# OpenGene/gencore

Measured on AMD Instinct MI355X. Metric: consensus read-pairs/sec (whole node) + clustering HBM GB/s vs roofline, higher is better.
Workload: dtype u8

## Files before the change

### gencore_amd/csrc/engine.hip

```cpp
#include <hip/hip_runtime.h>
#include <hip/hip_ext.h>
#include <cstdio>
#include <cstdlib>
#include <algorithm>
#include <cstring>
#include <ctime>
#include <string>
#include <vector>

#include "gce_kernels.hpp"
#include "gce_pair2.hpp"
#include "gce_vote.hpp"
#include "gce_deep.hpp"
#include "gce_output.hpp"
#include "gce_depth.hpp"
#include "gce_inflate.hpp"
#include "gce_deflate.hpp"

namespace {

static thread_local double t_alloc_s = 0.0; static thread_local long t_alloc_n = 0; static thread_local size_t t_alloc_bytes = 0;
static inline double mono_s() { struct timespec ts; clock_gettime(CLOCK_MONOTONIC, &ts); return (double)ts.tv_sec + 1e-9 * (double)ts.tv_nsec; }
long long g_dev_live = 0, g_dev_peak = 0;
static int64_t g_pass_idx_ctr[4] = {0, 0, 0, 0};
// ... 680 lines not shown
    }
    p.n_ref = nref; p.ref_data = e->d_ref_ptr.as<const uint8_t *>(); p.ref_len = e->d_ref_len.as<int64_t>(); p.ref_win = win.empty() ? nullptr : e->d_ref_win.as<int64_t>();

    Work w{};
    const int64_t n_sblk = (N + SB_READS - 1) / SB_READS;
    w.n_sblk = n_sblk;
    const int64_t max_events = e->have_tick ? (int64_t)e->h_ev_tid.size() + 2 : (p.tick_offset % p.period + N) / p.period + 2;
    w.max_events = (int)max_events;
    uint64_t T = ((uint64_t)n1 + (uint64_t)n1 / 4 + 2 * SCAN_TILE - 1) / SCAN_TILE * SCAN_TILE;
    w.tsize = T; w.tinv = 1.0 / (double)T;
    {
        uint64_t genome = 0; for (uint32_t v : e->target_len) genome += v;
        const uint64_t qmax = (genome * TAB_WAYS + TAB_WAYS) / T + 1;
        int cb = 1; while (cb < 33 && (1ull << cb) <= (uint64_t)N + 1024) cb++;
        int qb = 1; while (qb < 52 && (1ull << qb) <= qmax) qb++;
        p.nw_cb = cb; p.nw_bd = 62 - cb - qb; p.nw_ok = !e->target_len.empty() && p.nw_bd >= 1;
        if (p.nw_bd > 40) p.nw_bd = 40;
    }
    const size_t qual_bytes = hb.qual_bytes ? hb.qual_bytes : 1;
    const size_t nsb1 = (size_t)(n_sblk > 0 ? n_sblk : 1);
#define ENS(buf, bytes) HIPCHK(e->buf.ensure(bytes))
    ENS(uinfo, n1 * 8); ENS(rdesc, n1 * sizeof(ReadDescP)); ENS(spatch, n1 * 4); ENS(slot, n1 * 4 + 16); ENS(score, qual_bytes + 64);
    ENS(out_flag, n1 + 144);        ENS(nmx, n1 * 4); ENS(orec, n1 * sizeof(OutRec)); ENS(out_index, n1 * 4);
    ENS(lrec, nsb1 * SB_READS * sizeof(LeadRec)); ENS(lout, nsb1 * SB_READS * sizeof(LeadOut));
    ENS(bhdr, nsb1 * sizeof(BlkHdr)); ENS(blk_base, nsb1 * 4);
    ENS(ev_tid, (size_t)max_events * 4); ENS(ev_pos, (size_t)max_events * 4); ENS(ev_read, (size_t)max_events * 4);
    ENS(table, T * sizeof(TabEntry)); ENS(toff, T * 4);
    ENS(k64, n1 * 24); ENS(members, n1 * 4); ENS(sorted, n1 * 4); ENS(pl, n1 * 4); ENS(pr, n1 * 4); ENS(pu, n1 * 4); ENS(pg, n1 * 4); ENS(gpl, n1 * 4); ENS(gpr, n1 * 4);
    ENS(grp_begin, n1 * 4); ENS(grp_n, n1 * 4); ENS(slow_list, n1 * 4 + 64);
    w.slow_list = e->slow_list.as<uint32_t>();
    ENS(deep_list, (n1 / 64 + 64) * 16); w.deep_list = e->deep_list.p;
    const unsigned nblk_N = cdiv(n1, SCAN_TILE);
    ENS(scan_part, std::max<size_t>(2 * nsb1, (size_t)2 * nblk_N) * 8 + 16);     ENS(si, sizeof(StreamInfo));
    w.uinfo = e->uinfo.as<uint64_t>(); w.rdesc = e->rdesc.as<ReadDescP>(); w.spatch = e->spatch.as<uint32_t>();
    w.slot = e->slot.as<uint32_t>(); w.score = e->score.as<int8_t>();
    w.out_flag = e->out_flag.as<uint8_t>(); w.nmx = e->nmx.as<uint32_t>(); w.orec = e->orec.as<OutRec>(); w.out_index = e->out_index.as<uint32_t>();
    w.lrec = e->lrec.as<LeadRec>(); w.lout = e->lout.as<LeadOut>(); w.bhdr = e->bhdr.as<BlkHdr>(); w.blk_base = e->blk_base.as<uint32_t>();
    w.ev_tid = e->ev_tid.as<int32_t>(); w.ev_pos = e->ev_pos.as<int32_t>(); w.ev_read = e->ev_read.as<uint32_t>();
    w.tab = e->table.as<TabEntry>(); w.toff = e->toff.as<uint32_t>();
    w.k64 = e->k64.as<uint64_t>(); w.members = e->members.as<uint32_t>(); w.sorted = e->sorted.as<uint32_t>(); w.pl = e->pl.as<uint32_t>(); w.pr = e->pr.as<uint32_t>();
    w.pu = e->pu.as<uint32_t>(); w.pg = e->pg.as<uint32_t>(); w.gpl = e->gpl.as<uint32_t>(); w.gpr = e->gpr.as<uint32_t>();
    w.grp_begin = e->grp_begin.as<uint32_t>(); w.grp_n = e->grp_n.as<uint32_t>();
    w.scan_part = e->scan_part.as<uint64_t>(); w.si = e->si.as<StreamInfo>();
    ENS(cl_ikey, n1 * 4); ENS(cl_start, n1 * 4); ENS(cl_n, n1 * 4);
    w.cl_ikey = e->cl_ikey.as<uint32_t>(); w.cl_start = e->cl_start.as<uint32_t>(); w.cl_n = e->cl_n.as<uint32_t>();

    StreamInfo init{}; init.first_unmapped = NONE32; init.err_key = ~0ull; init.lq_min = 0x7FFFFFFF; init.lq_max = -1;
    if (e->have_tick) { init.n_events = init.n_events_a = (int)e->h_ev_tid.size(); }
    HIPCHK(hipMemcpyAsync(e->si.p, &init, sizeof init, hipMemcpyHostToDevice, e->stream));
    if (e->have_tick && !e->h_ev_tid.empty()) {
        HIPCHK(hipMemcpyAsync(e->ev_tid.p, e->h_ev_tid.data(), e->h_ev_tid.size() * 4, hipMemcpyHostToDevice, e->stream));
        HIPCHK(hipMemcpyAsync(e->ev_pos.p, e->h_ev_pos.data(), e->h_ev_pos.size() * 4, hipMemcpyHostToDevice, e->stream));
    }
    hipStream_t s = e->stream;
    if (!e->tab_clean || e->tab_clean_ptr != e->table.p || e->tab_clean_cap != e->table.cap) {
        HIPCHK(hipMemsetAsync(e->table.p, 0, e->table.cap, s));
        e->tab_clean_ptr = e->table.p; e->tab_clean_cap = e->table.cap;
    }
    e->tab_clean = false;
    HIPCHK(hipEventRecord(e->ev[EV_START], s));
    HIPCHK(hipMemsetAsync(e->out_flag.p, 0, n1, s));
    if (N > 0) LAUNCH_EV(k_cluster, dim3((unsigned)n_sblk), dim3(SB_T), s, e->ev[EV_CLUSTER], b, p, w);
#ifdef CL_PROF
    if (N > 0) {
        StreamInfo hs; (void)hipStreamSynchronize(s); (void)hipMemcpy(&hs, e->si.p, sizeof hs, hipMemcpyDeviceToHost);
        static const char *nm[3] = {"key records + keys", "LDS leaders", "stores"};
        const double blocks = (double)hs.prof[15];
        fprintf(stderr, "k_cluster phases, mean per block (us), %.0f blocks:", blocks);
        for (int k = 0; k < 3; k++) fprintf(stderr, " %s %.2f;", nm[k], blocks ? hs.prof[k] / blocks / 100.0 : 0.0);
        fprintf(stderr, "\n");
    }
#endif
    if (N <= 0) HIPCHK(hipEventRecord(e->ev[EV_CLUSTER], s));
    CANARY("EV_CLUSTER");
    if (N > 0) {
        if (!e->have_tick) {
            hipLaunchKernelGGL(k_blk_scan, dim3(1), dim3(1024), 0, s, w, p);
            hipLaunchKernelGGL(k_events, dim3(cdiv(max_events, EV_T / 64)), dim3(EV_T), 0, s, b, p, w);
        }
        const unsigned nb4 = cdiv(n_sblk, 4);
        hipLaunchKernelGGL(k_leaders, dim3(nb4), dim3(256), 0, s, b, p, w);
        hipLaunchKernelGGL(k_num_reduce, dim3(nb4), dim3(256), 0, s, w, p.nw_cb);
        hipLaunchKernelGGL(k_scan_partials, dim3(1), dim3(1024), 0, s, w.scan_part, (uint64_t)nb4, &w.si->n_clusters, (unsigned long long *)nullptr);
        hipLaunchKernelGGL(k_num_apply, dim3(nb4), dim3(256), 0, s, w);
        LAUNCH_EV(k_scatter, dim3((unsigned)n_sblk), dim3(SB_T), s, e->ev[EV_CSR], N, w);
    } else HIPCHK(hipEventRecord(e->ev[EV_CSR], s));
    CANARY("EV_CSR");
    unsigned long long si_seq1 = 0;
    if ((rc = read_si_begin(e, &si_seq1)) != GCE_OK) return rc;
    if (N > 0) {
#ifndef GCE_DESCRIBE_BLOCKS
#define GCE_DESCRIBE_BLOCKS 32768
#endif
        const int64_t n_tiles = (N + 255) / 256;
        int tpb = (int)((n_tiles + GCE_DESCRIBE_BLOCKS - 1) / GCE_DESCRIBE_BLOCKS); if (tpb < 1) tpb = 1;
        LAUNCH_EV(k_describe, dim3(cdiv(n_tiles, tpb)), dim3(256), s, e->ev[EV_DESCRIBE], b, p, w, tpb);
    } else HIPCHK(hipEventRecord(e->ev[EV_DESCRIBE], s));
    CANARY("EV_DESCRIBE");
    if ((rc = read_si_end(e, si_seq1)) != GCE_OK) return rc;
    HIPCHK(hipGetLastError());
    e->tab_clean = true;
    const uint32_t C = (uint32_t)e->h_si.n_clusters;
    const size_t c1 = C ? C : 1;
    ENS(cl_npairs, c1 * 4); ENS(cl_ngroups, c1 * 4); ENS(cl_gbase, c1 * 4); ENS(cl_nresult, c1 * 4); ENS(cl_hasumi, c1); ENS(cl_tier, c1);
    w.cl_npairs = e->cl_npairs.as<uint32_t>(); w.cl_ngroups = e->cl_ngroups.as<uint32_t>(); w.cl_gbase = e->cl_gbase.as<uint32_t>();
    w.cl_nresult = e->cl_nresult.as<uint32_t>(); w.cl_hasumi = e->cl_hasumi.as<uint8_t>(); w.cl_tier = e->cl_tier.as<uint8_t>();
    uint32_t NG = 0;
    bool si_behind_describe = false;
    if (C > 0 && e->dev_error == 0) {
        ENS(left_list, c1 * 4 + 64); w.left_list = e->left_list.as<uint32_t>();
        ENS(pf_flag, c1 + 64); ENS(pf_list, c1 * 4); ENS(pq_flag, c1 + 64); ENS(pq_list, c1 * 4); ENS(p16_flag, c1 + 64); ENS(p16_list, c1 * 4);
        w.pf_flag = e->pf_flag.as<uint8_t>(); w.pf_list = e->pf_list.as<uint32_t>(); w.pq_flag = e->pq_flag.as<uint8_t>(); w.pq_list = e->pq_list.as<uint32_t>(); w.p16_flag = e->p16_flag.as<uint8_t>(); w.p16_list = e->p16_list.as<uint32_t>();
        const bool pair_classes = (double)N > 10.0 * (double)C;
        if (!pair_classes) fill_many(s, {FillSeg{e->pf_flag.p, c1, 0u, 0u}, FillSeg{e->pq_flag.p, c1, 0u, 0u}});
        const unsigned nbc = cdiv(C, SCAN_TILE);
        auto compact = [&](uint8_t *flag, uint32_t *list, unsigned long long *count) {
            hipLaunchKernelGGL(k_flag_reduce, dim3(nbc), dim3(256), 0, s, (const uint8_t *)flag, (uint64_t)C, w.scan_part);
            hipLaunchKernelGGL(k_scan_partials, dim3(1), dim3(1024), 0, s, w.scan_part, (uint64_t)nbc, count, (unsigned long long *)nullptr);
            hipLaunchKernelGGL(k_flag_apply, dim3(nbc), dim3(256), 0, s, (const uint8_t *)flag, (uint64_t)C, (const uint64_t *)w.scan_part, list);
        };
#ifdef PS_STOP
        {
            hipEvent_t a_, b_, c_; (void)hipEventCreate(&a_); (void)hipEventCreate(&b_); (void)hipEventCreate(&c_);
            (void)hipEventRecord(a_, s);
            hipLaunchKernelGGL(k_pairing_sub<16>, dim3(cdiv(C, 4 * WAVES_PER_BLOCK)), dim3(256), 0, s, b, p, w, C, (const uint32_t *)nullptr, (const unsigned long long *)nullptr, w.pq_flag, 0);
            (void)hipEventRecord(b_, s);
            hipLaunchKernelGGL(k_pairing_sub<32>, dim3(cdiv(C, 2 * WAVES_PER_BLOCK)), dim3(256), 0, s, b, p, w, C, (const uint32_t *)nullptr, (const unsigned long long *)nullptr, w.pf_flag, 0);
            (void)hipEventRecord(c_, s); (void)hipEventSynchronize(c_);
            float m1 = 0, m2 = 0; (void)hipEventElapsedTime(&m1, a_, b_); (void)hipEventElapsedTime(&m2, b_, c_);
            fprintf(stderr, "k_pairing_sub up to tick %d: <16> %.3f ms, <32> over ALL clusters %.3f ms\n", PS_STOP, m1, m2);
            return fail(e, GCE_ERR_INVALID, "experiment build");
        }
#endif
        ENS(pd_slab, PD_BIG_BLOCKS * PD_SLAB);
        if (pair_classes) {
            hipLaunchKernelGGL(k_pair_class_reduce, dim3(nbc), dim3(256), 0, s, (const uint32_t *)w.cl_n, C, w.scan_part);
            hipLaunchKernelGGL(k_scan_partials, dim3(1), dim3(1024), 0, s, w.scan_part, (uint64_t)nbc, &w.si->n_p16_items, &w.si->n_pq_items);
            hipLaunchKernelGGL(k_pair_class_apply, dim3(nbc), dim3(256), 0, s, (const uint32_t *)w.cl_n, C, (const uint64_t *)w.scan_part, w.p16_list, w.pq_list, w.pf_list, w.si);
            static const bool tiers_aux = getenv("GCE_NO_AUX_STREAM") == nullptr;
            hipStream_t s2 = s;
            if (tiers_aux) {
                if ((rc = aux_ready(e)) != GCE_OK) return rc;
                s2 = e->aux_stream;
                HIPCHK(hipEventRecord(e->aux_ev[0], s));
                HIPCHK(hipStreamWaitEvent(s2, e->aux_ev[0], 0));
            }
            hipLaunchKernelGGL(k_pairing_fast, dim3(2048), dim3(256), 0, s2, b, p, w, C, (const uint32_t *)w.pf_list);
            hipLaunchKernelGGL(k_pairing_deep<false>, dim3(256), dim3(PD_T), 0, s2, b, p, w, (uint8_t *)nullptr);
            if (tiers_aux) HIPCHK(hipEventRecord(e->aux_ev[1], s2));
            hipLaunchKernelGGL(k_pairing_sub<16>, dim3(cdiv(C, 4 * WAVES_PER_BLOCK)), dim3(256), 0, s, b, p, w, C, (const uint32_t *)w.p16_list, (const unsigned long long *)&w.si->n_p16_items, w.pq_flag, 1);
            hipLaunchKernelGGL(k_pairing_sub<32>, dim3(cdiv(C, 2 * WAVES_PER_BLOCK)), dim3(256), 0, s, b, p, w, C, (const uint32_t *)w.pq_list, (const unsigned long long *)&w.si->n_pq_items, w.pf_flag, 1);
            if (tiers_aux) HIPCHK(hipStreamWaitEvent(s, e->aux_ev[1], 0));
        } else {
            hipLaunchKernelGGL(k_pairing_sub<16>, dim3(cdiv(C, 4 * WAVES_PER_BLOCK)), dim3(256), 0, s, b, p, w, C, (const uint32_t *)nullptr, (const unsigned long long *)nullptr, w.pq_flag, 0);
            compact(w.pq_flag, w.pq_list, &w.si->n_pq_items);
            hipLaunchKernelGGL(k_pairing_sub<32>, dim3(cdiv(C, 2 * WAVES_PER_BLOCK)), dim3(256), 0, s, b, p, w, C, (const uint32_t *)w.pq_list, (const unsigned long long *)&w.si->n_pq_items, w.pf_flag, 0);
            compact(w.pf_flag, w.pf_list, &w.si->n_pf_items);
            hipLaunchKernelGGL(k_pairing_fast, dim3(2048), dim3(256), 0, s, b, p, w, C, (const uint32_t *)w.pf_list);
            hipLaunchKernelGGL(k_pairing_deep<false>, dim3(256), dim3(PD_T), 0, s, b, p, w, (uint8_t *)nullptr);
        }
        hipLaunchKernelGGL(k_pairing_deep<true>, dim3(PD_BIG_BLOCKS), dim3(PD_T), 0, s, b, p, w, e->pd_slab.as<uint8_t>());
        hipLaunchKernelGGL(k_pairing_slow<0>, dim3(1024), dim3(256), 0, s, b, p, w);
        hipLaunchKernelGGL(k_pairing_slow<1>, dim3(1024, 16), dim3(256), 0, s, b, p, w);
        hipLaunchKernelGGL(k_pairing_slow<2>, dim3(1024), dim3(256), 0, s, b, p, w);
        const unsigned nblk_C = cdiv(C, SCAN_TILE);
        hipLaunchKernelGGL(k_scan_reduce, dim3(nblk_C), dim3(256), 0, s, (const uint32_t *)w.cl_ngroups, (uint64_t)C, w.scan_part);
        hipLaunchKernelGGL(k_scan_partials, dim3(1), dim3(1024), 0, s, w.scan_part, (uint64_t)nblk_C, &w.si->n_pairs , &w.si->n_groups);
        hipLaunchKernelGGL(k_u32_apply, dim3(nblk_C), dim3(256), 0, s, (const uint32_t *)w.cl_ngroups, w.cl_gbase, (uint64_t)C, (const uint64_t *)w.scan_part);
        ENS(gl_cluster, n1 * 4); ENS(g_begin, n1 * 4); ENS(g_np, n1 * 4); ENS(gw, n1 * 8); ENS(g_wbase, n1 * 4);
        const size_t vb_cap = ((VB_MINW + 3) * n1) / VB_W + 8;
        ENS(vb_start, vb_cap * 4);
        w.gl_cluster = e->gl_cluster.as<uint32_t>(); w.g_begin = e->g_begin.as<uint32_t>(); w.g_np = e->g_np.as<uint32_t>();
        w.gw = e->gw.as<uint64_t>(); w.g_wbase = e->g_wbase.as<uint32_t>(); w.vb_start = e->vb_start.as<uint32_t>();
        HIPCHK(hipMemsetAsync(e->vb_start.p, 0xFF, vb_cap * 4, s));
        hipLaunchKernelGGL(k_group_fill, dim3(cdiv(C, 256)), dim3(256), 0, s, w, C, p.skip_low_complexity_thr, (uint32_t)VB_W, (uint32_t)VB_MINW);
        hipLaunchKernelGGL(k_u64_reduce, dim3(nblk_N), dim3(256), 0, s, (const uint64_t *)w.gw, (const unsigned long long *)&w.si->n_groups, w.scan_part);
        hipLaunchKernelGGL(k_u64_partials, dim3(1), dim3(1024), 0, s, w.scan_part, (const unsigned long long *)&w.si->n_groups, &w.si->vote_weight);
        LAUNCH_EV(k_vote_batches, dim3(nblk_N), dim3(256), s, e->ev[EV_PAIRING], w, (const unsigned long long *)&w.si->n_groups, (const uint64_t *)w.scan_part);
        CANARY("EV_PAIRING");
        if ((rc = read_si(e)) != GCE_OK) return rc;
// ... 350 lines not shown
```

### gencore_amd/csrc/gce_cluster.hpp

```cpp
#pragma once

#ifndef SB_T
#define SB_T 512
#endif
#ifndef SB_U
#define SB_U 2
#endif
#define SB_READS (SB_T * SB_U)
#define SB_LDS_SLOTS (2 * SB_READS)
#define SB_OFF_BITS (SB_READS == 1024 ? 10 : 9)
static_assert(SB_READS == 512 || SB_READS == 1024, "LeadRec.info packs a place and a count of SB_READS");

struct __attribute__((aligned(16))) LeadRec { unsigned long long kw; uint32_t info, runlen; };
static_assert(sizeof(LeadRec) == 16, "LeadRec must stay 16 bytes");
#define LI_ODD (1u << 22)
struct __attribute__((aligned(8))) BlkHdr { uint32_t n_lead, n_clu; };
struct __attribute__((aligned(8))) LeadOut { uint32_t h, rb; };
#define LO_OWNER 0x80000000u

__device__ __forceinline__ uint32_t d_thr_mode(uint32_t ikey, const StreamInfo *si, const DevParams &p) {
    uint32_t inst = ikey & 0x7FFFFFFFu, seg_b = ikey >> 31;
    if (!seg_b) {
        if ((int)(inst + 1) <= si->n_events_a) return THR_PROPER;
        if (si->first_unmapped != NONE32) return THR_UNPROPER;
        return p.trailing_flush ? THR_PROPER : THR_UNPROPER;
    }
    return ((int)(inst + 1) <= si->n_events) ? THR_PROPER : THR_NEVER;
}

struct __attribute__((aligned(16))) TabEntry { unsigned long long key; unsigned long long ic; };
static_assert(sizeof(TabEntry) == 16, "TabEntry must stay 16 bytes");
#define TAB_OCC (1ull << 63)
#define TAB_EXO (1ull << 62)

#define TAB_WAYS 8
__device__ __forceinline__ uint64_t d_tab_index(const ClusterKey &k, uint32_t ikey, const DevParams &p) {
    uint64_t g = (k.tid >= 0 && k.tid < p.n_targets && p.target_cum) ? p.target_cum[k.tid] : (uint64_t)(uint32_t)k.tid * 0x9E3779B97F4A7C15ull;
    uint64_t m = ((uint64_t)k.right * 0x165667B19E3779F9ull) ^ ((uint64_t)ikey * 0xD6E8FEB86659FD93ull);
    m ^= m >> 29;
    return (((g + (uint64_t)(uint32_t)k.left) & 0x0000FFFFFFFFFFFFull) * TAB_WAYS) | (m & (TAB_WAYS - 1));
}
__device__ __forceinline__ unsigned long long d_pack_key(const ClusterKey &k, const DevParams &p) {
    const long long delta1 = k.right - (long long)k.left + 1;
    const int bd = 62 - p.key_bt - p.key_bl;
    if (k.tid >= 0 && ((uint64_t)(uint32_t)k.tid >> p.key_bt) == 0 && k.left >= 0 && ((uint64_t)(uint32_t)k.left >> p.key_bl) == 0 &&
        delta1 >= 0 && bd > 0 && ((uint64_t)delta1 >> bd) == 0)
        return TAB_OCC | (uint64_t)(uint32_t)k.tid | ((uint64_t)(uint32_t)k.left << p.key_bt) | ((uint64_t)delta1 << (p.key_bt + p.key_bl));
    return 0ull;
}
__device__ __forceinline__ ClusterKey d_unpack_key(unsigned long long kw, const DevParams &p) {
    ClusterKey k;
    k.tid = (int32_t)(kw & ((1ull << p.key_bt) - 1ull));
    k.left = (int32_t)((kw >> p.key_bt) & ((1ull << p.key_bl) - 1ull));
    const long long delta1 = (long long)((kw & ~(TAB_OCC | TAB_EXO)) >> (p.key_bt + p.key_bl));
    k.right = (long long)k.left + delta1 - 1;
    return k;
}
__device__ __forceinline__ unsigned long long d_exotic_key(uint32_t ikey, uint32_t read) {
    return TAB_OCC | TAB_EXO | ((uint64_t)((ikey & 0x1FFFFFFFu) | ((ikey >> 31) << 29)) << 32) | read;
}

#ifdef CL_PROF
#define CL_TICK(k) do { if (threadIdx.x == 0 && (blockIdx.x & 31) == 0) { const unsigned long long now_ = wall_clock64(); atomicAdd(&w.si->prof[k], now_ - t_prev_); t_prev_ = now_; } } while (0)
#else
#define CL_TICK(k) do { } while (0)
#endif
__global__ __launch_bounds__(SB_T, 2048 / SB_T) void k_cluster(DevBatch b, DevParams p, Work w) {
    __shared__ uint32_t s_slot[SB_LDS_SLOTS];
    __shared__ unsigned long long s_kw[SB_READS];
    __shared__ uint32_t s_cnt[SB_READS];
    __shared__ uint16_t s_num[SB_READS];
    __shared__ uint32_t s_wcnt[SB_U][SB_T / 64];
    __shared__ uint32_t s_nlead;
    __shared__ uint32_t s_unm[SB_T / 64];
    const int lane = lane_id(), wv = threadIdx.x >> 6;
#ifdef CL_PROF
    unsigned long long t_prev_ = wall_clock64();
    if (threadIdx.x == 0 && (blockIdx.x & 31) == 0) atomicAdd(&w.si->prof[15], 1ull);
#endif
    int64_t idx[SB_U]; gce_core k[SB_U]; int2 pv[SB_U];
#pragma unroll
    for (int u = 0; u < SB_U; u++) {
        idx[u] = ((int64_t)blockIdx.x * SB_U + u) * SB_T + threadIdx.x;
        union { gce_core c; uint4 q[2]; } t;
        t.q[0] = make_uint4(0, 0, 0, 0); t.q[1] = t.q[0];
        pv[u] = make_int2(-1, -1);
        if (idx[u] < b.n) {
            const uint4 *src = reinterpret_cast<const uint4 *>(b.core + idx[u]); t.q[0] = src[0]; t.q[1] = src[1];
            if (idx[u] > 0) pv[u] = *reinterpret_cast<const int2 *>(b.core + idx[u] - 1);
        }
        k[u] = t.c;
    }
    for (int q = threadIdx.x; q < SB_LDS_SLOTS; q += SB_T) s_slot[q] = 0;
    if (threadIdx.x == 0) s_nlead = 0;
    bool cl[SB_U], odd[SB_U], unm = false; unsigned long long m[SB_U], kw[SB_U];
#pragma unroll
    for (int u = 0; u < SB_U; u++) {
        const bool in = idx[u] < b.n;
        const uint8_t c = in ? d_classify(k[u]) : (uint8_t)CLS_DROP;
        cl[u] = c == CLS_CLUSTERED;
        bool unm_u = false;
        if (in) {
            if (idx[u] > 0 && (k[u].tid < pv[u].x || (k[u].tid == pv[u].x && k[u].pos < pv[u].y)) && k[u].tid >= 0 && k[u].pos >= 0)
                raise_error(w.si, GCE_ERR_UNSORTED, (uint32_t)idx[u]);
            if (k[u].tid < 0 || k[u].pos < 0) unm_u = true;
            if (c == CLS_BYPASS) w.out_flag[idx[u]] = 2;
        }
        if (__any(unm_u)) {
            unm = true;
            const unsigned int v = (unsigned int)wave_min((int)((unm_u ? (unsigned int)idx[u] : NONE32) ^ 0x80000000u)) ^ 0x80000000u;
            if (lane == 0 && v < *(volatile unsigned int *)&w.si->first_unmapped) atomicMin(&w.si->first_unmapped, v);
        }
        m[u] = __ballot(cl[u]);
        if (lane == 0) s_wcnt[u][wv] = (uint32_t)__popcll(m[u]);
        kw[u] = 0ull; odd[u] = false;
        if (cl[u]) {
            const ClusterKey key = d_key(k[u], p);
            odd[u] = key.right < (long long)k[u].pos;
            kw[u] = d_pack_key(key, p);
        }
        const int id = u * SB_T + threadIdx.x;
        s_kw[id] = kw[u]; s_cnt[id] = 0u;
    }
    {
        const unsigned long long um = __ballot(unm);
        if (lane == 0) s_unm[wv] = um != 0ull;
    }
    __syncthreads();
    int any_unm = 0;
#pragma unroll
    for (int q = 0; q < SB_T / 64; q++) any_unm |= (int)s_unm[q];
    CL_TICK(0);
    int leader[SB_U]; uint32_t lrank[SB_U];
#pragma unroll
    for (int u = 0; u < SB_U; u++) {
        leader[u] = -1; lrank[u] = 0;
        if (cl[u]) {
            const int id = u * SB_T + threadIdx.x;
            leader[u] = id;
            if (kw[u] != 0ull && !odd[u] && !any_unm) {
                uint32_t hs = ((uint32_t)kw[u] ^ (uint32_t)(kw[u] >> 29)) * 0x9E3779B1u;
                hs = (hs ^ (hs >> 15)) & (SB_LDS_SLOTS - 1);
                for (;;) {
                    const uint32_t old = atomicCAS(&s_slot[hs], 0u, (uint32_t)id + 1u);
                    if (old == 0u) break;
                    const int L = (int)old - 1;
                    if (s_kw[L] == kw[u]) { leader[u] = L; break; }
                    hs = (hs + 1) & (SB_LDS_SLOTS - 1);
                }
            }
            lrank[u] = atomicAdd(&s_cnt[leader[u]], 1u);
            if (leader[u] == id) s_num[id] = (uint16_t)atomicAdd(&s_nlead, 1u);
        }
    }
    __syncthreads();
    CL_TICK(1);
    uint32_t front = 0;
#pragma unroll
    for (int u = 0; u < SB_U; u++) {
        const int id = u * SB_T + threadIdx.x;
        uint32_t inblock = front + (uint32_t)lanes_below(m[u]);
#pragma unroll
        for (int q = 0; q < SB_T / 64; q++) { const uint32_t c = s_wcnt[u][q]; inblock += q < wv ? c : 0u; front += c; }
        if (idx[u] < b.n) {
            if (cl[u]) {
                w.slot[idx[u]] = (uint32_t)s_num[leader[u]] | lrank[u] << 16;
                if (leader[u] == id) {
                    union { LeadRec r; uint4 q; } o;
                    o.r.kw = kw[u]; o.r.info = (uint32_t)id | inblock << SB_OFF_BITS | (odd[u] ? LI_ODD : 0u); o.r.runlen = s_cnt[id];
                    *reinterpret_cast<uint4 *>(w.lrec + (size_t)blockIdx.x * SB_READS + s_num[id]) = o.q;
                }
            } else w.slot[idx[u]] = NONE32;
        }
    }
    if (threadIdx.x == 0) { BlkHdr h; h.n_lead = s_nlead; h.n_clu = front; w.bhdr[blockIdx.x] = h; }
    CL_TICK(2);
}

__global__ __launch_bounds__(1024) void k_blk_scan(Work w, DevParams p) {
    __shared__ unsigned int s_w[16], s_l[16];
    const int lane = lane_id(), wv = threadIdx.x >> 6;
    const int64_t per_w = ((w.n_sblk + 15) / 16 + 255) / 256 * 256, w0 = per_w * wv, w1 = min(w0 + per_w, w.n_sblk);
    auto load4 = [&](int64_t i, unsigned int (&c)[4], unsigned int &nl) {
        if (i + 3 < w1) {
            const uint4 q0 = reinterpret_cast<const uint4 *>(w.bhdr + i)[0], q1 = reinterpret_cast<const uint4 *>(w.bhdr + i)[1];
            c[0] = q0.y; c[1] = q0.w; c[2] = q1.y; c[3] = q1.w; nl += q0.x + q0.z + q1.x + q1.z;
        } else {
#pragma unroll
            for (int k = 0; k < 4; k++) { c[k] = 0; if (i + k < w1) { const BlkHdr h = w.bhdr[i + k]; c[k] = h.n_clu; nl += h.n_lead; } }
        }
    };
    unsigned int v = 0, nl = 0;
    for (int64_t i = w0 + 4 * lane; i < w1; i += 256) { unsigned int c[4]; load4(i, c, nl); v += c[0] + c[1] + c[2] + c[3]; }
    v = (unsigned int)wave_sum((int)v); nl = (unsigned int)wave_sum((int)nl);
    if (lane == 0) { s_w[wv] = v; s_l[wv] = nl; }
    __syncthreads();
    unsigned int carry = 0, tot = 0; unsigned long long leaders = 0;
#pragma unroll
    for (int k = 0; k < 16; k++) { const unsigned int t = s_w[k]; tot += t; carry += k < wv ? t : 0u; leaders += s_l[k]; }
    for (int64_t i0 = w0; i0 < w1; i0 += 256) {
        const int64_t i = i0 + 4 * lane;
        unsigned int c[4], dummy = 0; load4(i, c, dummy);
        const unsigned int sum = c[0] + c[1] + c[2] + c[3];
        const unsigned int x = (unsigned int)wave_scan_incl((int)sum);
        unsigned int run = carry + x - sum;
#pragma unroll
        for (int k = 0; k < 4; k++) { if (i + k < w1) w.blk_base[i + k] = run; run += c[k]; }
        carry += (unsigned int)__builtin_amdgcn_readlane((int)x, 63);
    }
    if (threadIdx.x == 0) {
        unsigned long long total = tot;
        w.si->n_clustered = total;
        w.si->n_leaders = leaders;
        long long per_ = p.period;
        long long e = (p.tick_offset + (long long)total) / per_ - p.tick_offset / per_;
        w.si->n_events = (int)(e < w.max_events ? e : w.max_events);
        if (e > w.max_events) raise_error(w.si, GCE_ERR_INVALID, 0);
    }
}

#define EV_T 1024
__global__ __launch_bounds__(EV_T) void k_events(DevBatch b, DevParams p, Work w) {
    __shared__ int s_a;
    if (threadIdx.x == 0) s_a = 0;
    __syncthreads();
    const int j = (int)((blockIdx.x * blockDim.x + threadIdx.x) >> 6), lane = lane_id();
    const int E = w.si->n_events;
    if (j < E) {
        const long long per = p.period;
        const long long gt = (p.tick_offset / per + (j + 1)) * per;
        const unsigned int t = (unsigned int)(gt - p.tick_offset);
        int64_t lo = 0, hi = w.n_sblk - 1;
        while (lo < hi) {
            const int64_t step = (hi - lo + 63) / 64, probe = lo + (int64_t)(lane + 1) * step;
            const bool below = probe <= hi && w.blk_base[probe] < t;
            const int k = __popcll(__ballot(below));
            hi = min(hi, lo + (int64_t)(k + 1) * step - 1);
            lo = lo + (int64_t)k * step;
        }
        unsigned int need = t - w.blk_base[lo];
        const int64_t i0 = lo * SB_READS, end = min(b.n, i0 + SB_READS);
        int64_t i = end;
        bool clq[SB_READS / 64];
#pragma unroll
        for (int q = 0; q < SB_READS / 64; q++) {
            const int64_t idx = i0 + 64 * q + lane;
            clq[q] = idx < end && w.slot[idx] != NONE32;
        }
#pragma unroll
        for (int q = 0; q < SB_READS / 64; q++) {
            const bool cl = clq[q];
            const unsigned long long m = __ballot(cl);
            const unsigned int cnt = (unsigned int)__popcll(m);
            if (need <= cnt) {
                const unsigned long long hit = __ballot(cl && (unsigned int)__popcll(m & ((1ull << lane) - 1ull)) + 1u == need);
                i = i0 + 64 * q + (__ffsll((long long)hit) - 1);
                break;
            }
            need -= cnt;
// ... 141 lines not shown
}
__device__ __forceinline__ uint64_t tab_elem(const uint32_t *cnt, uint64_t h, uint64_t n) {
    if (h >= n) return 0;
    uint32_t c = cnt[h];
    return ((uint64_t)(c > 0) << 32) | c;
}
__global__ __launch_bounds__(256) void k_scan_reduce(const uint32_t *cnt, uint64_t n, uint64_t *part) {
    __shared__ uint64_t s[4];
    uint64_t base = (uint64_t)blockIdx.x * SCAN_TILE, v = 0;
    for (int k = 0; k < SCAN_TILE / 256; k++) v += tab_elem(cnt, base + k * 256 + threadIdx.x, n);
    v = (uint64_t)wave_sum64((long long)v);
    if (lane_id() == 0) s[threadIdx.x >> 6] = v;
    __syncthreads();
    if (threadIdx.x == 0) part[blockIdx.x] = s[0] + s[1] + s[2] + s[3];
}
__global__ __launch_bounds__(1024) void k_scan_partials(uint64_t *part, uint64_t nparts, unsigned long long *total_hi, unsigned long long *total_lo) {
    __shared__ uint64_t s_w[2][16];
    const int lane = lane_id(), wv = threadIdx.x >> 6;
    uint64_t carry = 0;
    int it = 0;
    for (uint64_t base = 0; base < nparts; base += 8192, it ^= 1) {
        const uint64_t i0 = base + 8 * (uint64_t)threadIdx.x;
        uint64_t c[8], v = 0;
#pragma unroll
        for (int k = 0; k < 8; k++) { c[k] = i0 + k < nparts ? part[i0 + k] : 0; v += c[k]; }
        uint64_t x = v;
        for (int o = 1; o < 64; o <<= 1) { uint64_t t = (uint64_t)__shfl_up((long long)x, o); if (lane >= o) x += t; }
        if (lane == 63) s_w[it][wv] = x;
        __syncthreads();
        uint64_t woff = 0, tot = 0;
#pragma unroll
        for (int k = 0; k < 16; k++) { const uint64_t t = s_w[it][k]; tot += t; woff += k < wv ? t : 0ull; }
        uint64_t run = carry + woff + x - v;
#pragma unroll
        for (int k = 0; k < 8; k++) { if (i0 + k < nparts) part[i0 + k] = run; run += c[k]; }
        carry += tot;
    }
    if (threadIdx.x == 0) { *total_hi = carry >> 32; if (total_lo) *total_lo = carry & 0xFFFFFFFFull; }
}
__global__ __launch_bounds__(256) void k_num_apply(Work w) {
    const int lane = lane_id();
    const int64_t blk = (int64_t)blockIdx.x * (blockDim.x >> 6) + (threadIdx.x >> 6);
    if (blk >= w.n_sblk) return;
    const uint32_t nl = w.bhdr[blk].n_lead;
    uint64_t carry = w.scan_part[blockIdx.x];
    for (int q = 0; q < (int)(threadIdx.x >> 6); q++) carry += w.scan_part[gridDim.x + blk - (threadIdx.x >> 6) + q];
    for (uint32_t k0 = 0; k0 < nl; k0 += 64) {
        const uint32_t kq = k0 + (uint32_t)lane;
        uint64_t v = 0, ic = 0; uint32_t h = 0;
        if (kq < nl) {
            const size_t LR = (size_t)blk * SB_READS + kq;
            const LeadOut o = w.lout[LR];
            if (o.rb & LO_OWNER) { h = o.h; ic = w.lrec[LR].kw; v = (1ull << 32) | (uint32_t)ic; }
        }
        uint64_t x = v;
        for (int o = 1; o < 64; o <<= 1) { uint64_t t = (uint64_t)__shfl_up((long long)x, o); if (lane >= o) x += t; }
        if (v) {
            const uint64_t ex = carry + x - v;
            const uint32_t cid = (uint32_t)(ex >> 32);
            w.cl_start[cid] = (uint32_t)ex; w.cl_n[cid] = (uint32_t)v; w.cl_ikey[cid] = (uint32_t)(ic >> 32); w.toff[h] = (uint32_t)ex;
        }
        carry += rl64(x, 63);
    }
}
__global__ __launch_bounds__(SB_T) void k_scatter(int64_t n, Work w) {
    __shared__ uint32_t s_dst[SB_READS];
    const int64_t blk = blockIdx.x;
    const uint32_t nl = w.bhdr[blk].n_lead;
    uint32_t v[SB_U];
#pragma unroll
    for (int u = 0; u < SB_U; u++) { const int64_t i = (blk * SB_U + u) * SB_T + threadIdx.x; v[u] = i < n ? w.slot[i] : NONE32; }
    for (uint32_t kq = threadIdx.x; kq < nl; kq += SB_T) {
        const LeadOut o = w.lout[(size_t)blk * SB_READS + kq];
        s_dst[kq] = w.toff[o.h] + (o.rb & ~LO_OWNER);
        if (o.rb & LO_OWNER) *reinterpret_cast<uint4 *>(&w.tab[o.h]) = make_uint4(0, 0, 0, 0);
    }
    __syncthreads();
#pragma unroll
    for (int u = 0; u < SB_U; u++) {
        const int64_t i = (blk * SB_U + u) * SB_T + threadIdx.x;
        if (v[u] != NONE32) w.members[s_dst[v[u] & 0xFFFFu] + (v[u] >> 16)] = (uint32_t)i;
    }
}

#ifndef DESC_WPE
#define DESC_WPE 8
#endif
__global__ __launch_bounds__(256, DESC_WPE) void k_describe(DevBatch b, DevParams p, Work w, int tiles_per_block) {
    __shared__ long long s_stat[WAVES_PER_BLOCK][6];
    long long st[6] = {0, 0, 0, 0, 0, 0};
    int lqmin = 0x7FFFFFFF, lqmax = -1;
    const int lane = lane_id(), wv = threadIdx.x >> 6;
    for (int cb = 0; cb < tiles_per_block; cb++) {
        const int64_t i = ((int64_t)blockIdx.x * tiles_per_block + cb) * 256 + threadIdx.x;
        if (i < b.n) {
            union { gce_core c; uint4 q[2]; } t; const uint4 *src = reinterpret_cast<const uint4 *>(b.core + i); t.q[0] = src[0]; t.q[1] = src[1];
            const gce_core k = t.c;
            const uint8_t c = d_classify(k);
            bool mapped = k.tid >= 0;
            const int nmv = b.nm[i]; const bool has_nm = b.nm_type[i] != 0;
            int mism = (mapped && has_nm) ? nmv : 0;
            w.nmx[i] = ((uint32_t)nmv << 1) | (has_nm ? 1u : 0u);
            st[0] += 1; st[1] += k.l_qseq; st[4] += mism;
            if (!mapped) { st[2] += 1; st[3] += k.l_qseq; }
            if (mism > 0) st[5] += 1;
            if (c != CLS_DROP) { lqmin = min(lqmin, k.l_qseq); lqmax = max(lqmax, k.l_qseq); }
            if (c == CLS_CLUSTERED) {
                const uint32_t *cg = b.cigar + b.cigar_off[i];
                const uint32_t c0w = k.n_cigar ? cg[0] : 0;
                int mo_ = 0, ml_ = 0;
                if (k.n_cigar == 1) ml_ = cig_op(c0w) == 0 ? cig_len(c0w) : 0;
                else d_first_m(cg, k.n_cigar, mo_, ml_);
                if (k.l_qseq > 65535) raise_error(w.si, GCE_ERR_INVALID, (uint32_t)i);
                if (p.ref_win && k.isize != 0 && k.tid < p.n_ref && p.ref_data[k.tid]) {
                    const int64_t rl = k.n_cigar == 1 ? (int64_t)cig_len(c0w) * consumes_ref(cig_op(c0w)) : (int64_t)d_cigar_rlen(cg, k.n_cigar);
                    const int64_t end_in = min((int64_t)k.pos + rl, p.ref_len[k.tid]);
                    if ((int64_t)k.pos < p.ref_win[2 * k.tid] || end_in > p.ref_win[2 * k.tid + 1]) raise_error(w.si, GCE_ERR_REF_WINDOW, (uint32_t)i);
                }
                store_desc(w.rdesc, (uint64_t)i, b.seq_off[i], b.qual_off[i], c0w, k.pos, k.isize != 0, k.l_qseq, mo_, ml_, k.n_cigar, k.tid, k.n_cigar > 1 ? cg[k.n_cigar - 1] : c0w);
                const char *src2; uint8_t hm = 0;
                if (b.mi && b.mi_off[i] != 0xFFFFFFFFFFFFFFFFull) { src2 = b.mi + b.mi_off[i]; hm = 1; }
                else src2 = b.qname + b.qname_off[i];
                int s0, l0;
                if (!d_umi_slice(src2, p, s0, l0, hm ? -1 : (int)k.l_qname - 1)) { raise_error(w.si, GCE_ERR_UMI_PARSE, (uint32_t)i); s0 = 0; l0 = 0; }
                if (l0 > UINFO_MAXLEN) { raise_error(w.si, GCE_ERR_UMI_PARSE, (uint32_t)i); l0 = 0; }
                w.uinfo[i] = uinfo_pack((hm ? b.mi_off[i] : b.qname_off[i]) + (uint64_t)s0, hm != 0, k.l_qname, l0);
            }
        }
    }
    for (int k = 0; k < 6; k++) { long long v = wave_sum64(st[k]); if (lane == 0) s_stat[wv][k] = v; }
    lqmin = wave_min(lqmin); lqmax = wave_max(lqmax);
    if (lane == 0) {
        if (lqmin < *(volatile int *)&w.si->lq_min) atomicMin(&w.si->lq_min, lqmin);
        if (lqmax > *(volatile int *)&w.si->lq_max) atomicMax(&w.si->lq_max, lqmax);
    }
    __syncthreads();
    if (threadIdx.x < 6) {
        long long v = s_stat[0][threadIdx.x] + s_stat[1][threadIdx.x] + s_stat[2][threadIdx.x] + s_stat[3][threadIdx.x];
        if (v) atomicAdd((unsigned long long *)&w.si->pre_slot[blockIdx.x & (GCE_PRE_SLOTS - 1)][threadIdx.x], (unsigned long long)v);
    }
}
```

Baseline: 1.806 billion.

## Fuse per-read describe pass into k_cluster and drop k_describe kernel

The per-read describe work (NM packing, stats, CIGAR first-M, ref-window check, rdesc store, UMI slice) moves into the tail of k_cluster, which already holds each read's core record in registers. This removes a separate kernel launch and a second full read of the core array. The stats reduction becomes per-wave atomics into pre_slot. The read_si handshake is moved earlier in the launch sequence. Launch bounds change from 2048/SB_T to a tunable CL_WPE (8). The extra work raises register pressure in k_cluster and may lower its occupancy.

```diff
diff --git a/gencore_amd/csrc/engine.hip b/gencore_amd/csrc/engine.hip
--- a/gencore_amd/csrc/engine.hip
+++ b/gencore_amd/csrc/engine.hip
@@ -786,20 +786,16 @@
         hipLaunchKernelGGL(k_leaders, dim3(nb4), dim3(256), 0, s, b, p, w);
         hipLaunchKernelGGL(k_num_reduce, dim3(nb4), dim3(256), 0, s, w, p.nw_cb);
         hipLaunchKernelGGL(k_scan_partials, dim3(1), dim3(1024), 0, s, w.scan_part, (uint64_t)nb4, &w.si->n_clusters, (unsigned long long *)nullptr);
+    }
+    unsigned long long si_seq1 = 0;
+    if ((rc = read_si_begin(e, &si_seq1)) != GCE_OK) return rc;
+    if (N > 0) {
+        const unsigned nb4 = cdiv(n_sblk, 4);
         hipLaunchKernelGGL(k_num_apply, dim3(nb4), dim3(256), 0, s, w);
         LAUNCH_EV(k_scatter, dim3((unsigned)n_sblk), dim3(SB_T), s, e->ev[EV_CSR], N, w);
     } else HIPCHK(hipEventRecord(e->ev[EV_CSR], s));
     CANARY("EV_CSR");
-    unsigned long long si_seq1 = 0;
-    if ((rc = read_si_begin(e, &si_seq1)) != GCE_OK) return rc;
-    if (N > 0) {
-#ifndef GCE_DESCRIBE_BLOCKS
-#define GCE_DESCRIBE_BLOCKS 32768
-#endif
-        const int64_t n_tiles = (N + 255) / 256;
-        int tpb = (int)((n_tiles + GCE_DESCRIBE_BLOCKS - 1) / GCE_DESCRIBE_BLOCKS); if (tpb < 1) tpb = 1;
-        LAUNCH_EV(k_describe, dim3(cdiv(n_tiles, tpb)), dim3(256), s, e->ev[EV_DESCRIBE], b, p, w, tpb);
-    } else HIPCHK(hipEventRecord(e->ev[EV_DESCRIBE], s));
+    HIPCHK(hipEventRecord(e->ev[EV_DESCRIBE], s));
     CANARY("EV_DESCRIBE");
     if ((rc = read_si_end(e, si_seq1)) != GCE_OK) return rc;
     HIPCHK(hipGetLastError());
diff --git a/gencore_amd/csrc/gce_cluster.hpp b/gencore_amd/csrc/gce_cluster.hpp
--- a/gencore_amd/csrc/gce_cluster.hpp
+++ b/gencore_amd/csrc/gce_cluster.hpp
@@ -60,12 +60,47 @@
     return TAB_OCC | TAB_EXO | ((uint64_t)((ikey & 0x1FFFFFFFu) | ((ikey >> 31) << 29)) << 32) | read;
 }
 
+struct DescAcc { long long st[6]; int lqmin, lqmax; };
+__device__ __forceinline__ void d_describe(const DevBatch &b, const DevParams &p, const Work &w, int64_t i, const gce_core &k, uint8_t c, DescAcc &a) {
+    const bool mapped = k.tid >= 0;
+    const int nmv = b.nm[i]; const bool has_nm = b.nm_type[i] != 0;
+    const int mism = (mapped && has_nm) ? nmv : 0;
+    w.nmx[i] = ((uint32_t)nmv << 1) | (has_nm ? 1u : 0u);
+    a.st[0] += 1; a.st[1] += k.l_qseq; a.st[4] += mism;
+    if (!mapped) { a.st[2] += 1; a.st[3] += k.l_qseq; }
+    if (mism > 0) a.st[5] += 1;
+    if (c != CLS_DROP) { a.lqmin = min(a.lqmin, k.l_qseq); a.lqmax = max(a.lqmax, k.l_qseq); }
+    if (c != CLS_CLUSTERED) return;
+    const uint32_t *cg = b.cigar + b.cigar_off[i];
+    const uint32_t c0w = k.n_cigar ? cg[0] : 0;
+    int mo_ = 0, ml_ = 0;
+    if (k.n_cigar == 1) ml_ = cig_op(c0w) == 0 ? cig_len(c0w) : 0;
+    else d_first_m(cg, k.n_cigar, mo_, ml_);
+    if (k.l_qseq > 65535) raise_error(w.si, GCE_ERR_INVALID, (uint32_t)i);
+    if (p.ref_win && k.isize != 0 && k.tid < p.n_ref && p.ref_data[k.tid]) {
+        const int64_t rl = k.n_cigar == 1 ? (int64_t)cig_len(c0w) * consumes_ref(cig_op(c0w)) : (int64_t)d_cigar_rlen(cg, k.n_cigar);
+        const int64_t end_in = min((int64_t)k.pos + rl, p.ref_len[k.tid]);
+        if ((int64_t)k.pos < p.ref_win[2 * k.tid] || end_in > p.ref_win[2 * k.tid + 1]) raise_error(w.si, GCE_ERR_REF_WINDOW, (uint32_t)i);
+    }
+    store_desc(w.rdesc, (uint64_t)i, b.seq_off[i], b.qual_off[i], c0w, k.pos, k.isize != 0, k.l_qseq, mo_, ml_, k.n_cigar, k.tid, k.n_cigar > 1 ? cg[k.n_cigar - 1] : c0w);
+    const char *src2; uint8_t hm = 0;
+    if (b.mi && b.mi_off[i] != 0xFFFFFFFFFFFFFFFFull) { src2 = b.mi + b.mi_off[i]; hm = 1; }
+    else src2 = b.qname + b.qname_off[i];
+    int s0, l0;
+    if (!d_umi_slice(src2, p, s0, l0, hm ? -1 : (int)k.l_qname - 1)) { raise_error(w.si, GCE_ERR_UMI_PARSE, (uint32_t)i); s0 = 0; l0 = 0; }
+    if (l0 > UINFO_MAXLEN) { raise_error(w.si, GCE_ERR_UMI_PARSE, (uint32_t)i); l0 = 0; }
+    w.uinfo[i] = uinfo_pack((hm ? b.mi_off[i] : b.qname_off[i]) + (uint64_t)s0, hm != 0, k.l_qname, l0);
+}
+
 #ifdef CL_PROF
 #define CL_TICK(k) do { if (threadIdx.x == 0 && (blockIdx.x & 31) == 0) { const unsigned long long now_ = wall_clock64(); atomicAdd(&w.si->prof[k], now_ - t_prev_); t_prev_ = now_; } } while (0)
 #else
 #define CL_TICK(k) do { } while (0)
 #endif
-__global__ __launch_bounds__(SB_T, 2048 / SB_T) void k_cluster(DevBatch b, DevParams p, Work w) {
+#ifndef CL_WPE
+#define CL_WPE 8
+#endif
+__global__ __launch_bounds__(SB_T, CL_WPE) void k_cluster(DevBatch b, DevParams p, Work w) {
     __shared__ uint32_t s_slot[SB_LDS_SLOTS];
     __shared__ unsigned long long s_kw[SB_READS];
     __shared__ uint32_t s_cnt[SB_READS];
@@ -175,6 +210,21 @@
     }
     if (threadIdx.x == 0) { BlkHdr h; h.n_lead = s_nlead; h.n_clu = front; w.bhdr[blockIdx.x] = h; }
     CL_TICK(2);
+    DescAcc da = {{0, 0, 0, 0, 0, 0}, 0x7FFFFFFF, -1};
+#pragma unroll
+    for (int u = 0; u < SB_U; u++)
+        if (idx[u] < b.n) d_describe(b, p, w, idx[u], k[u], d_classify(k[u]), da);
+    da.lqmin = wave_min(da.lqmin); da.lqmax = wave_max(da.lqmax);
+    if (lane == 0) {
+        if (da.lqmin < *(volatile int *)&w.si->lq_min) atomicMin(&w.si->lq_min, da.lqmin);
+        if (da.lqmax > *(volatile int *)&w.si->lq_max) atomicMax(&w.si->lq_max, da.lqmax);
+    }
+    const int slot = (int)((blockIdx.x * (SB_T / 64) + wv) & (GCE_PRE_SLOTS - 1));
+#pragma unroll
+    for (int q = 0; q < 6; q++) {
+        const long long v = wave_sum64(da.st[q]);
+        if (lane == 0 && v) atomicAdd((unsigned long long *)&w.si->pre_slot[slot][q], (unsigned long long)v);
+    }
 }
 
 __global__ __launch_bounds__(1024) void k_blk_scan(Work w, DevParams p) {
@@ -482,61 +532,3 @@
         if (v[u] != NONE32) w.members[s_dst[v[u] & 0xFFFFu] + (v[u] >> 16)] = (uint32_t)i;
     }
 }
-
-#ifndef DESC_WPE
-#define DESC_WPE 8
-#endif
-__global__ __launch_bounds__(256, DESC_WPE) void k_describe(DevBatch b, DevParams p, Work w, int tiles_per_block) {
-    __shared__ long long s_stat[WAVES_PER_BLOCK][6];
-    long long st[6] = {0, 0, 0, 0, 0, 0};
-    int lqmin = 0x7FFFFFFF, lqmax = -1;
-    const int lane = lane_id(), wv = threadIdx.x >> 6;
-    for (int cb = 0; cb < tiles_per_block; cb++) {
-        const int64_t i = ((int64_t)blockIdx.x * tiles_per_block + cb) * 256 + threadIdx.x;
-        if (i < b.n) {
-            union { gce_core c; uint4 q[2]; } t; const uint4 *src = reinterpret_cast<const uint4 *>(b.core + i); t.q[0] = src[0]; t.q[1] = src[1];
-            const gce_core k = t.c;
-            const uint8_t c = d_classify(k);
-            bool mapped = k.tid >= 0;
-            const int nmv = b.nm[i]; const bool has_nm = b.nm_type[i] != 0;
-            int mism = (mapped && has_nm) ? nmv : 0;
-            w.nmx[i] = ((uint32_t)nmv << 1) | (has_nm ? 1u : 0u);
-            st[0] += 1; st[1] += k.l_qseq; st[4] += mism;
-            if (!mapped) { st[2] += 1; st[3] += k.l_qseq; }
-            if (mism > 0) st[5] += 1;
-            if (c != CLS_DROP) { lqmin = min(lqmin, k.l_qseq); lqmax = max(lqmax, k.l_qseq); }
-            if (c == CLS_CLUSTERED) {
-                const uint32_t *cg = b.cigar + b.cigar_off[i];
-                const uint32_t c0w = k.n_cigar ? cg[0] : 0;
-                int mo_ = 0, ml_ = 0;
-                if (k.n_cigar == 1) ml_ = cig_op(c0w) == 0 ? cig_len(c0w) : 0;
-                else d_first_m(cg, k.n_cigar, mo_, ml_);
-                if (k.l_qseq > 65535) raise_error(w.si, GCE_ERR_INVALID, (uint32_t)i);
-                if (p.ref_win && k.isize != 0 && k.tid < p.n_ref && p.ref_data[k.tid]) {
-                    const int64_t rl = k.n_cigar == 1 ? (int64_t)cig_len(c0w) * consumes_ref(cig_op(c0w)) : (int64_t)d_cigar_rlen(cg, k.n_cigar);
-                    const int64_t end_in = min((int64_t)k.pos + rl, p.ref_len[k.tid]);
-                    if ((int64_t)k.pos < p.ref_win[2 * k.tid] || end_in > p.ref_win[2 * k.tid + 1]) raise_error(w.si, GCE_ERR_REF_WINDOW, (uint32_t)i);
-                }
-                store_desc(w.rdesc, (uint64_t)i, b.seq_off[i], b.qual_off[i], c0w, k.pos, k.isize != 0, k.l_qseq, mo_, ml_, k.n_cigar, k.tid, k.n_cigar > 1 ? cg[k.n_cigar - 1] : c0w);
-                const char *src2; uint8_t hm = 0;
-                if (b.mi && b.mi_off[i] != 0xFFFFFFFFFFFFFFFFull) { src2 = b.mi + b.mi_off[i]; hm = 1; }
-                else src2 = b.qname + b.qname_off[i];
-                int s0, l0;
-                if (!d_umi_slice(src2, p, s0, l0, hm ? -1 : (int)k.l_qname - 1)) { raise_error(w.si, GCE_ERR_UMI_PARSE, (uint32_t)i); s0 = 0; l0 = 0; }
-                if (l0 > UINFO_MAXLEN) { raise_error(w.si, GCE_ERR_UMI_PARSE, (uint32_t)i); l0 = 0; }
-                w.uinfo[i] = uinfo_pack((hm ? b.mi_off[i] : b.qname_off[i]) + (uint64_t)s0, hm != 0, k.l_qname, l0);
-            }
-        }
-    }
-    for (int k = 0; k < 6; k++) { long long v = wave_sum64(st[k]); if (lane == 0) s_stat[wv][k] = v; }
-    lqmin = wave_min(lqmin); lqmax = wave_max(lqmax);
-    if (lane == 0) {
-        if (lqmin < *(volatile int *)&w.si->lq_min) atomicMin(&w.si->lq_min, lqmin);
-        if (lqmax > *(volatile int *)&w.si->lq_max) atomicMax(&w.si->lq_max, lqmax);
-    }
-    __syncthreads();
-    if (threadIdx.x < 6) {
-        long long v = s_stat[0][threadIdx.x] + s_stat[1][threadIdx.x] + s_stat[2][threadIdx.x] + s_stat[3][threadIdx.x];
-        if (v) atomicAdd((unsigned long long *)&w.si->pre_slot[blockIdx.x & (GCE_PRE_SLOTS - 1)][threadIdx.x], (unsigned long long)v);
-    }
-}
```

Result: no change. 1.824 billion, median of 6 (+1.0%).
